# GregVS/Racing-SLAM

Measured on AMD Instinct MI355X. Metric: match+triangulate+local-BA passes/sec @ 2k kpts/frame, 20-KF×10k-pt window, higher is better.
Workload: dtype u8 Hamming (match), f64 (DLT SVD, BA), f32 (gates)

## Files before the change

racing-slam_amd/csrc/common.h:

```cpp
#pragma once
#include <hip/hip_runtime.h>
#include <stdint.h>
#include <stdio.h>
#include <string.h>

#include <string>
#include <vector>

#include "../../include/rsgpu.h"
#include "dev_array.h"

#define RS_WAVE 64

struct rs_prof_slot {
    char name[32];
    int launches;
    std::vector<hipEvent_t> ev;
};

struct rs_arena {
    char* base = nullptr;
    size_t cap = 0, used = 0;
    std::vector<void*> retired;
};
// ... 4 lines not shown
    hipStream_t stream = nullptr;
    std::string err;
    void* ws = nullptr;
    size_t ws_bytes = 0;
    int32_t* grp_zero_ptr = nullptr;
    int grp_zero_n = 0;
    size_t ws_dirty_hi = 0;
    void* pinned = nullptr;
    size_t pinned_bytes = 0;
    rs_arena stage_dev, stage_pin;
    std::vector<rs_pending_download> stage_down;
    bool prof_on = false;
    std::vector<rs_prof_slot> prof;
    void* comm = nullptr;
    int n_ranks = 1;
    int rank = 0;
    struct rs_local_group* local = nullptr;
    void* ba_cache = nullptr;
    const void* ba_trace = nullptr;
    int ba_trace_n = 0;
    int ba_stats[8] = {0, 0, 0, 0, 0, 0, 0, 0};
    int ba_item = 0;
    int ba_batch_item = 0;
    int ba_band_mode = 0;
    int ba_s_replicas = 0;
    int ba_handoff_timeout_us = 4000;
    const double* ba_cams = nullptr;
    int ba_cams_n = 0;
    int ba_sets = 0;
    int n_cu = 256;
    int ba_fuse_mode = 0;
    int k2_mode = 0;
    int k2_grid = 1;
    int ba_imu_mode = 0;
    int ba_batch_mode = 0;
    int bow_score_mode = 0;
    int loop_verify_streams = 0;
    int gftt_round_launches = 12;
    std::vector<rs_context*> batch_lanes;
    std::vector<hipStream_t> batch_streams;
    rs_dev_array<unsigned long long> prop;
    hipEvent_t sync_ev = nullptr;
    void* tri_pin = nullptr;
    int tri_ticket = 0;
    rs_dev_array<uint2> k1_top;
};

struct rs_frame {
    rs_context* ctx = nullptr;
    int n = 0;
    rs_dev_block block;
    rs_pin_block pin;
    float* d_kp = nullptr; uint8_t* d_desc = nullptr; int32_t* d_kd = nullptr;
    uint8_t* d_matched = nullptr;
    void* d_packed = nullptr;
    int kd_root = -1;
    int cap = 0;
    uint32_t* d_rank = nullptr;
    int32_t* d_n = nullptr;
    int32_t* h_n = nullptr;
    int32_t* d_kp_point = nullptr;
    rs_dev_array<unsigned char> grid;
    int grid_w = 0, grid_h = 0;
    bool grid_built = false;
    bool finite = false;
};
// ... 131 lines not shown
```

racing-slam_amd/csrc/context.hip:

```cpp
#include <dlfcn.h>
#include <stdarg.h>
#include <stdlib.h>

#include "common.h"

int rs_fail(rs_context* ctx, int code, const char* fmt, ...)
{
    char buf[512];
    va_list ap;
    va_start(ap, fmt);
    vsnprintf(buf, sizeof buf, fmt, ap);
    va_end(ap);
    if (ctx) ctx->err = buf;
    else fprintf(stderr, "rsgpu: %s\n", buf);
    return code;
}

extern "C" int rs_abi_version(void) { return RSGPU_ABI_VERSION; }

extern "C" int rs_context_create(int device_id, rs_context** out)
{
    if (!out) return RS_ERR_INVALID;
    *out = nullptr;
    int n = 0;
// ... 109 lines not shown
    if (strcmp(name, "ba_item_landmarks") == 0) {
        if (value != 0 && (value < 32 || value > 64 || value % 8)) return rs_fail(ctx, RS_ERR_INVALID, "ba_item_landmarks must be 0 (default) or 32, 40, 48, 56, 64");
        ctx->ba_item = value;
        return RS_OK;
    }
    if (strcmp(name, "ba_batch_item_landmarks") == 0) {
        if (value != 0 && (value < 32 || value > 64 || value % 8)) return rs_fail(ctx, RS_ERR_INVALID, "ba_batch_item_landmarks must be 0 (default) or 32, 40, 48, 56, 64");
        ctx->ba_batch_item = value;
        return RS_OK;
    }
    if (strcmp(name, "ba_band_mode") == 0) {
        if (value < 0 || value > 2) return rs_fail(ctx, RS_ERR_INVALID, "ba_band_mode must be 0 (banded factorisation where the reduced matrix is block-banded), 1 (always the general blocked one) or 2 (banded, one workgroup instead of two sides)");
        ctx->ba_band_mode = value;
        return RS_OK;
    }
    if (strcmp(name, "ba_s_replicas") == 0) {
        if (value != 0 && value != 1 && value != 2 && value != 4 && value != 8) return rs_fail(ctx, RS_ERR_INVALID, "ba_s_replicas must be 0 (default), 1, 2, 4 or 8");
        ctx->ba_s_replicas = value;
        return RS_OK;
    }
    if (strcmp(name, "ba_handoff_timeout_us") == 0) {
        if (value < 1 || value > 1000000) return rs_fail(ctx, RS_ERR_INVALID, "ba_handoff_timeout_us must be 1 .. 1000000");
        ctx->ba_handoff_timeout_us = value;
        return RS_OK;
    }
    if (strcmp(name, "k2_mode") == 0) {
        if (value < 0 || value > 1) return rs_fail(ctx, RS_ERR_INVALID, "k2_mode must be 0 (eight lanes per map point where possible) or 1 (one lane per point)");
        ctx->k2_mode = value;
        return RS_OK;
    }
    if (strcmp(name, "k2_grid") == 0) {
        if (value < 0 || value > 1) return rs_fail(ctx, RS_ERR_INVALID, "k2_grid must be 1 (the cell-grid kernel where the frame has a usable grid) or 0 (never)");
        ctx->k2_grid = value;
        return RS_OK;
    }
    if (strcmp(name, "ba_batch_mode") == 0) {
        if (value < 0 || value > 1) return rs_fail(ctx, RS_ERR_INVALID, "ba_batch_mode must be 0 (grid where possible) or 1 (lanes)");
        ctx->ba_batch_mode = value;
        return RS_OK;
    }
    if (strcmp(name, "bow_score_mode") == 0) {
        if (value < 0 || value > 1) return rs_fail(ctx, RS_ERR_INVALID, "bow_score_mode must be 0 (dense word table) or 1 (binary search)");
        ctx->bow_score_mode = value;
        return RS_OK;
    }
    if (strcmp(name, "loop_verify_streams") == 0) {
        if (value < 0 || value > 1) return rs_fail(ctx, RS_ERR_INVALID, "loop_verify_streams must be 0 (one child context per candidate) or 1 (the context stream)");
        ctx->loop_verify_streams = value;
        return RS_OK;
    }
    if (strcmp(name, "gftt_round_launches") == 0) {
        if (value < 0 || value > GFTT_ROUNDS_KNOB) return rs_fail(ctx, RS_ERR_INVALID, "gftt_round_launches must be 0 .. 12 (default 12)");
        ctx->gftt_round_launches = value;
        return RS_OK;
    }
    return rs_fail(ctx, RS_ERR_INVALID, "unknown option %s", name);
}

extern "C" int rs_context_synchronize(rs_context* ctx)
{
    if (!ctx) return RS_ERR_INVALID;
    RS_HIP(ctx, hipStreamSynchronize(ctx->stream));
    return RS_OK;
}

extern "C" const char* rs_last_error(const rs_context* ctx) { return ctx ? ctx->err.c_str() : "null context"; }
// ... 489 lines not shown
```

racing-slam_amd/csrc/tracks.hip:

```cpp
#include "point_core.h"

struct TrackParams {
    TriParams tri;
    float min_parallax_cosine;
    float rotation_factor;
    int kf_pose;
};

#define K6_TABLE_POSES 512
#define K6_BATCH 4

__global__ __launch_bounds__(64) void k6_tracks(const float2* __restrict__ track_uv, const uint8_t* __restrict__ skip,
                                               const int32_t* __restrict__ sight_ptr,
                                               const int32_t* __restrict__ sight_pose,
                                               const float2* __restrict__ sight_uv, const float* __restrict__ poses,
                                               int n_tracks, int n_table, TrackParams prm, uint8_t* __restrict__ status,
                                               float* __restrict__ xyz, float* __restrict__ parallax_cos,
                                               float* __restrict__ required_cos, const float* __restrict__ required_by_pose)
{
    extern __shared__ float kp_rows[];
    for (int i = threadIdx.x; i < n_table; i += blockDim.x) {
        float T[16], KP[12];
        load_pose(poses, i, T);
        projection_rows(prm.tri, T, KP);
#pragma unroll
        for (int k = 0; k < 12; k++) kp_rows[12 * i + k] = KP[k];
    }
    __syncthreads();
    const int t = blockIdx.x * blockDim.x + threadIdx.x;
    if (t >= n_tracks) return;
    const int s0 = sight_ptr[t], s1 = sight_ptr[t + 1];
    uint8_t st = 0;
    float X[3] = {0.f, 0.f, 0.f}, pc = 0.f, rc = 0.f;
    if (s1 > s0 && !(skip && skip[t])) {
        float Tf[16], Tk[16];
        load_pose(poses, sight_pose[s0], Tf);
        load_pose(poses, prm.kf_pose, Tk);
        const bool ok = dlt_one(sight_uv[s0], track_uv[t], Tf, Tk, prm.tri, X);
        if (ok) {
            bool consistent = true;
            if (n_table > 0) {
                for (int s = s0; s < s1 && consistent; s += K6_BATCH) {
                    int ip[K6_BATCH];
                    float2 px[K6_BATCH];
#pragma unroll
                    for (int u = 0; u < K6_BATCH; u++) { const int su = min(s + u, s1 - 1); ip[u] = sight_pose[su]; px[u] = sight_uv[su]; }
#pragma unroll
                    for (int u = 0; u < K6_BATCH; u++) {
                        float KP[12];
                        const int iu = min(max(ip[u], 0), n_table - 1);
#pragma unroll
                        for (int k = 0; k < 12; k++) KP[k] = kp_rows[12 * iu + k];
                        const float2 pr = project_rows_f32(KP, X);
                        const float dx = pr.x - px[u].x, dy = pr.y - px[u].y;
                        if (sqrtf(dx * dx + dy * dy) > prm.tri.max_reprojection_error) consistent = false;
                    }
                }
            } else
            for (int s = s0; s < s1; s++) {
                float Ts[16];
                load_pose(poses, sight_pose[s], Ts);
                const float2 pr = project_f32(prm.tri, Ts, X);
                const float2 px = sight_uv[s];
                const float dx = pr.x - px.x, dy = pr.y - px.y;
                if (sqrtf(dx * dx + dy * dy) > prm.tri.max_reprojection_error) { consistent = false; break; }
            }
            if (!consistent) {
                st = 2;
            } else {
                float cf[3], ck[3];
                camera_center_f32(Tf, cf);
                camera_center_f32(Tk, ck);
                float a[3] = {cf[0] - X[0], cf[1] - X[1], cf[2] - X[2]};
                float b[3] = {ck[0] - X[0], ck[1] - X[1], ck[2] - X[2]};
                normalize3f(a);
                normalize3f(b);
                float tr[3];
#pragma unroll
                for (int i = 0; i < 3; i++) {
                    const float rk[3] = {Tk[4 * i], Tk[4 * i + 1], Tk[4 * i + 2]};
                    const float rf[3] = {Tf[4 * i], Tf[4 * i + 1], Tf[4 * i + 2]};
                    tr[i] = dot3f(rk, rf);
                }
                const float trace = (tr[0] + tr[1]) + tr[2];
                float cosine = (trace - 1.0f) / 2.0f;
                cosine = cosine < -1.0f ? -1.0f : cosine;
                cosine = cosine > 1.0f ? 1.0f : cosine;
                st = 1;
                pc = dot3f(a, b);
                if (required_by_pose) {
                    rc = required_by_pose[sight_pose[s0]];
                } else {
                    const float turned = acosf(cosine);
                    const float need = cosf(prm.rotation_factor * turned);
                    rc = prm.min_parallax_cosine < need ? prm.min_parallax_cosine : need;
                }
            }
        }
    }
    status[t] = st;
    xyz[3 * (size_t)t + 0] = X[0]; xyz[3 * (size_t)t + 1] = X[1]; xyz[3 * (size_t)t + 2] = X[2];
    parallax_cos[t] = pc;
    required_cos[t] = rc;
}

#define K6B_CH 8
#define K6B_REJ_LDS 2048
#define K6B_FIELD 21

__device__ __forceinline__ bool k6_before(float kj, float ki, int j, int i)
{
    return (kj < ki) || (!(ki < kj) && !(kj < ki) && ((kj == kj) == (ki == ki)) && j < i) || ((kj == kj) && !(ki == ki));
}

__device__ __forceinline__ unsigned long long k6_block_exclusive_scan64(unsigned long long v, unsigned long long* total)
{
    __shared__ unsigned long long k6_scan_w[16];
    const int lane = threadIdx.x & 63, wave = threadIdx.x >> 6, nw = (blockDim.x + 63) >> 6;
    unsigned long long x = v;
#pragma unroll
    for (int off = 1; off < 64; off <<= 1) {
        const unsigned long long t = __shfl_up(x, off, 64);
        if (lane >= off) x += t;
    }
    if (lane == 63) k6_scan_w[wave] = x;
    __syncthreads();
    unsigned long long pre = 0, tot = 0;
    for (int w = 0; w < nw; w++) { const unsigned long long c = k6_scan_w[w]; if (w < wave) pre += c; tot += c; }
    __syncthreads();
    *total = tot;
    return pre + x - v;
}

template <int CH>
__device__ __forceinline__ void k6_select_held(const uint8_t* __restrict__ status, const float* __restrict__ pcs,
                                               const float* __restrict__ rcs, int lo, int hi, int min_new_points,
                                               int32_t* __restrict__ accepted, int32_t* __restrict__ inconsistent,
// ... 98 lines not shown
                                     const int32_t* d_sight_ptr, const int32_t* d_sight_pose,
                                     const float* d_sight_uv, const float* d_poses, int n_poses, int kf_pose,
                                     const float h_intrinsics[4], float any_parallax_cosine,
                                     float max_reprojection_error, float min_parallax_cosine,
                                     float rotation_parallax_factor, int min_new_points, uint8_t* d_status,
                                     float* d_xyz, float* d_parallax_cos, float* d_required_cos,
                                     int32_t* d_accepted, int32_t* d_inconsistent, int32_t* d_counts,
                                     const float* d_required_by_pose)
{
    if (!ctx) return RS_ERR_INVALID;
    if (n_tracks < 0 || n_poses < 0) return rs_fail(ctx, RS_ERR_INVALID, "negative size");
    if (!d_counts) return rs_fail(ctx, RS_ERR_INVALID, "null counts");
    RS_HIP(ctx, hipSetDevice(ctx->device));
    if (n_tracks == 0) {
        RS_HIP(ctx, hipMemsetAsync(d_counts, 0, 3 * sizeof(int32_t), ctx->stream));
        return RS_OK;
    }
    if (!d_track_uv || !d_sight_ptr || !d_sight_pose || !d_sight_uv || !d_poses || !h_intrinsics || !d_status ||
        !d_xyz || !d_parallax_cos || !d_required_cos || !d_accepted || !d_inconsistent)
        return rs_fail(ctx, RS_ERR_INVALID, "null pointer");
    if (kf_pose < 0 || kf_pose >= n_poses) return rs_fail(ctx, RS_ERR_INVALID, "key-frame pose index out of range");
    if ((uintptr_t)d_poses & 15) return rs_fail(ctx, RS_ERR_INVALID, "poses must be 16-byte aligned");
    void* ws = nullptr;
    int rc = rs_workspace(ctx, sizeof(int32_t) * (size_t)n_tracks, &ws);
    if (rc) return rc;
    TrackParams prm;
    prm.tri = {h_intrinsics[0], h_intrinsics[1], h_intrinsics[2], h_intrinsics[3], any_parallax_cosine, max_reprojection_error};
    prm.min_parallax_cosine = min_parallax_cosine;
    prm.rotation_factor = rotation_parallax_factor;
    prm.kf_pose = kf_pose;
    {
        rs_prof_scope ps(ctx, "K6_tracks");
        const int n_table = n_poses <= K6_TABLE_POSES ? n_poses : 0;
        hipLaunchKernelGGL(k6_tracks, dim3((n_tracks + 63) / 64), dim3(64), sizeof(float) * 12 * (size_t)n_table, ctx->stream,
                           (const float2*)d_track_uv, d_skip, d_sight_ptr, d_sight_pose, (const float2*)d_sight_uv, d_poses, n_tracks, n_table, prm,
                           d_status, d_xyz, d_parallax_cos, d_required_cos, d_required_by_pose);
    }
    {
        rs_prof_scope ps(ctx, "K6b_select");
        hipLaunchKernelGGL(k6_select, dim3(1), dim3(1024), 0, ctx->stream, d_status, d_parallax_cos, d_required_cos,
                           n_tracks, min_new_points, d_accepted, d_inconsistent, (int32_t*)ws, d_counts);
    }
    RS_HIP(ctx, hipGetLastError());
    return RS_OK;
}

__global__ __launch_bounds__(256) void k12_point_errors(const float* __restrict__ pos, const int32_t* __restrict__ obs_ptr,
                                                        const int32_t* __restrict__ obs_pose,
                                                        const float2* __restrict__ obs_uv, const float* __restrict__ poses,
                                                        int n_points, TriParams k, float max_mean_error,
                                                        float* __restrict__ mean_err, uint8_t* __restrict__ cull,
                                                        double* __restrict__ sums)
{
    const int p = blockIdx.x * blockDim.x + threadIdx.x;
    double esum = 0.0, ecnt = 0.0;
    if (p < n_points) {
        const float X[3] = {pos[3 * (size_t)p], pos[3 * (size_t)p + 1], pos[3 * (size_t)p + 2]};
        const int o0 = obs_ptr[p], o1 = obs_ptr[p + 1];
        const float err = point_error_sum_f32(k, poses, obs_pose, obs_uv, nullptr, X, o0, o1, &esum);
        const int cnt = o1 - o0;
        ecnt = (double)cnt;
        float mean;
        const bool c = point_cull_rule_f32(err, cnt, max_mean_error, &mean);
        mean_err[p] = mean;
        cull[p] = c ? 1 : 0;
    }
    esum = wave_sum_f64(esum);
// ... 186 lines not shown
```

racing-slam_amd/csrc/tri_core.h:

```cpp
#pragma once
#include "common.h"

struct TriParams {
    float fx, fy, cx, cy;
    float min_parallax_cosine, max_reprojection_error;
};

__device__ __forceinline__ double cv_hypot(double a, double b)
{
    a = fabs(a);
    b = fabs(b);
    if (a > b) { b /= a; return a * sqrt(1 + b * b); }
    if (b > 0) { a /= b; return b * sqrt(1 + a * a); }
    return 0;
}

__device__ __forceinline__ float dot3f(const float* a, const float* b) { return (a[0] * b[0] + a[1] * b[1]) + a[2] * b[2]; }

__device__ __forceinline__ void normalize3f(float* v)
{
    const float n = dot3f(v, v);
    if (n > 0.0f) {
        const float s = sqrtf(n);
        v[0] = v[0] / s; v[1] = v[1] / s; v[2] = v[2] / s;
    }
}

__device__ __forceinline__ float det3f(float a, float b, float c, float d, float e, float f, float g, float h, float i)
{
    return (a * (e * i - f * h) - b * (d * i - f * g)) + c * (d * h - e * g);
}

__device__ __forceinline__ void inverse_translation(const float* T, float* c)
{
    const float M0 = det3f(T[1], T[2], T[3], T[5], T[6], T[7], T[9], T[10], T[11]);
    const float M1 = det3f(T[0], T[2], T[3], T[4], T[6], T[7], T[8], T[10], T[11]);
    const float M2 = det3f(T[0], T[1], T[3], T[4], T[5], T[7], T[8], T[9], T[11]);
    const float M3 = det3f(T[0], T[1], T[2], T[4], T[5], T[6], T[8], T[9], T[10]);
    const float det = (-T[12] * M0 + T[13] * M1) + (-T[14] * M2 + T[15] * M3);
    c[0] = -M0 / det;
    c[1] = M1 / det;
    c[2] = -M2 / det;
}

__device__ __forceinline__ void projection_rows(const TriParams& k, const float* T, float* P)
{
#pragma unroll
    for (int j = 0; j < 4; j++) {
        P[0 * 4 + j] = (k.fx * T[0 * 4 + j] + 0.0f * T[1 * 4 + j]) + k.cx * T[2 * 4 + j];
        P[1 * 4 + j] = (0.0f * T[0 * 4 + j] + k.fy * T[1 * 4 + j]) + k.cy * T[2 * 4 + j];
        P[2 * 4 + j] = (0.0f * T[0 * 4 + j] + 0.0f * T[1 * 4 + j]) + 1.0f * T[2 * 4 + j];
    }
}

#define JACOBI_PAIR(i, j)                                                                      \
    {                                                                                          \
        double a = W[i], p = 0, b = W[j];                                                      \
        _Pragma("unroll") for (int k = 0; k < 4; k++) p += At[i][k] * At[j][k];                \
        if (!(fabs(p) <= eps * sqrt(a * b))) {                                                 \
            p *= 2;                                                                            \
            const double beta = a - b, gamma = cv_hypot(p, beta);                              \
            double c, s;                                                                       \
            if (beta < 0) {                                                                    \
                const double delta = (gamma - beta) * 0.5;                                     \
                s = sqrt(delta / gamma);                                                       \
                c = p / (gamma * s * 2);                                                       \
            } else {                                                                           \
                c = sqrt((gamma + beta) / (gamma * 2));                                        \
                s = p / (gamma * c * 2);                                                       \
            }                                                                                  \
            a = 0; b = 0;                                                                      \
            _Pragma("unroll") for (int k = 0; k < 4; k++) {                                    \
                const double t0 = c * At[i][k] + s * At[j][k];                                 \
                const double t1 = -s * At[i][k] + c * At[j][k];                                \
                At[i][k] = t0; At[j][k] = t1;                                                  \
                a += t0 * t0; b += t1 * t1;                                                    \
            }                                                                                  \
            W[i] = a; W[j] = b;                                                                \
            changed = true;                                                                    \
            _Pragma("unroll") for (int k = 0; k < 4; k++) {                                    \
                const double t0 = c * Vt[i][k] + s * Vt[j][k];                                 \
                const double t1 = -s * Vt[i][k] + c * Vt[j][k];                                \
                Vt[i][k] = t0; Vt[j][k] = t1;                                                  \
            }                                                                                  \
        }                                                                                      \
    }

__device__ __forceinline__ void load_pose(const float* __restrict__ poses, int idx, float* T)
{
    const float4* a = (const float4*)(poses + 16 * (size_t)idx);
#pragma unroll
    for (int r = 0; r < 4; r++) {
        const float4 v = a[r];
        T[4 * r] = v.x; T[4 * r + 1] = v.y; T[4 * r + 2] = v.z; T[4 * r + 3] = v.w;
    }
}

__device__ __forceinline__ float2 project_rows_f32(const float* KP, const float* X)
{
    float uvw[3];
#pragma unroll
    for (int i = 0; i < 3; i++)
        uvw[i] = (KP[4 * i] * X[0] + KP[4 * i + 1] * X[1]) + (KP[4 * i + 2] * X[2] + KP[4 * i + 3] * 1.0f);
    if (uvw[2] < 0.0f) return make_float2(-1.0f, -1.0f);
    return make_float2(uvw[0] / uvw[2], uvw[1] / uvw[2]);
}

__device__ __forceinline__ float2 project_f32(const TriParams& k, const float* T, const float* X)
{
    float KP[12];
    projection_rows(k, T, KP);
    return project_rows_f32(KP, X);
}

__device__ __forceinline__ void camera_center_f32(const float* T, float* c)
{
    const float t[3] = {T[3], T[7], T[11]};
#pragma unroll
    for (int i = 0; i < 3; i++) {
        const float a[3] = {-T[0 * 4 + i], -T[1 * 4 + i], -T[2 * 4 + i]};
        c[i] = dot3f(a, t);
    }
}

__device__ __forceinline__ double wave_sum_f64(double v)
{
#pragma unroll
    for (int off = 32; off > 0; off >>= 1) v += __shfl_xor(v, off, 64);
    return v;
}

__device__ __forceinline__ bool dlt_one(const float2 p1, const float2 p2, const float* T1, const float* T2,
                                        const TriParams& prm, float* Xout)
{
    double At[4][4], Vt[4][4], W[4];
    {
        float P1[12], P2[12];
        projection_rows(prm, T1, P1);
        projection_rows(prm, T2, P2);
#pragma unroll
        for (int k = 0; k < 4; k++) {
            At[k][0] = (double)p1.x * (double)P1[8 + k] - (double)P1[k];
            At[k][1] = (double)p1.y * (double)P1[8 + k] - (double)P1[4 + k];
            At[k][2] = (double)p2.x * (double)P2[8 + k] - (double)P2[k];
            At[k][3] = (double)p2.y * (double)P2[8 + k] - (double)P2[4 + k];
        }
    }
    const double eps = 2.220446049250313e-16 * 10;
#pragma unroll
    for (int r = 0; r < 4; r++) {
        double sd = 0;
#pragma unroll
        for (int k = 0; k < 4; k++) sd += At[r][k] * At[r][k];
        W[r] = sd;
#pragma unroll
        for (int k = 0; k < 4; k++) Vt[r][k] = (r == k) ? 1.0 : 0.0;
    }
    for (int iter = 0; iter < 30; iter++) {
        bool changed = false;
        JACOBI_PAIR(0, 1) JACOBI_PAIR(0, 2) JACOBI_PAIR(0, 3)
        JACOBI_PAIR(1, 2) JACOBI_PAIR(1, 3) JACOBI_PAIR(2, 3)
        if (!changed) break;
    }
#pragma unroll
    for (int r = 0; r < 4; r++) {
        double sd = 0;
#pragma unroll
        for (int k = 0; k < 4; k++) sd += At[r][k] * At[r][k];
        W[r] = sqrt(sd);
    }
#pragma unroll
    for (int a = 0; a < 3; a++) {
        int j = a;
#pragma unroll
        for (int k = a + 1; k < 4; k++)
            if (W[j] < W[k]) j = k;
#pragma unroll
        for (int k = a + 1; k < 4; k++) {
            if (j == k) {
                const double tw = W[a]; W[a] = W[k]; W[k] = tw;
#pragma unroll
                for (int m = 0; m < 4; m++) { const double tv = Vt[a][m]; Vt[a][m] = Vt[k][m]; Vt[k][m] = tv; }
            }
        }
    }
    const float h0 = (float)Vt[3][0], h1 = (float)Vt[3][1], h2 = (float)Vt[3][2], h3 = (float)Vt[3][3];
    float X[3] = {h0 / h3, h1 / h3, h2 / h3};
    Xout[0] = X[0]; Xout[1] = X[1]; Xout[2] = X[2];

    bool ok = true;
    float c1[3], c2[3];
#pragma unroll
    for (int r = 0; r < 3; r++) {
        c1[r] = (T1[4 * r] * X[0] + T1[4 * r + 1] * X[1]) + (T1[4 * r + 2] * X[2] + T1[4 * r + 3] * 1.0f);
        c2[r] = (T2[4 * r] * X[0] + T2[4 * r + 1] * X[1]) + (T2[4 * r + 2] * X[2] + T2[4 * r + 3] * 1.0f);
    }
    if (c1[2] < 0.0f || c2[2] < 0.0f) ok = false;
    float o1[3], o2[3];
    inverse_translation(T1, o1);
    inverse_translation(T2, o2);
    float a[3] = {o1[0] - X[0], o1[1] - X[1], o1[2] - X[2]};
    float b[3] = {o2[0] - X[0], o2[1] - X[1], o2[2] - X[2]};
    normalize3f(a);
    normalize3f(b);
    if (dot3f(a, b) > prm.min_parallax_cosine) ok = false;
    const float w1 = (0.0f * c1[0] + 0.0f * c1[1]) + 1.0f * c1[2];
    const float w2 = (0.0f * c2[0] + 0.0f * c2[1]) + 1.0f * c2[2];
    const float i1x = ((prm.fx * c1[0] + 0.0f * c1[1]) + prm.cx * c1[2]) / w1;
    const float i1y = ((0.0f * c1[0] + prm.fy * c1[1]) + prm.cy * c1[2]) / w1;
    const float i2x = ((prm.fx * c2[0] + 0.0f * c2[1]) + prm.cx * c2[2]) / w2;
    const float i2y = ((0.0f * c2[0] + prm.fy * c2[1]) + prm.cy * c2[2]) / w2;
    const float e1x = i1x - p1.x, e1y = i1y - p1.y, e2x = i2x - p2.x, e2y = i2y - p2.y;
    const float err1 = sqrtf(e1x * e1x + e1y * e1y);
    const float err2 = sqrtf(e2x * e2x + e2y * e2y);
    if (err1 > prm.max_reprojection_error || err2 > prm.max_reprojection_error) ok = false;
    return ok;
}
```

racing-slam_amd/csrc/triangulate.hip:

```cpp
#include "tri_core.h"

__device__ __forceinline__ void k4_triangulate_body(
    const float2* __restrict__ uv1, const float2* __restrict__ uv2, int n,
    const float* __restrict__ poses, const int32_t* __restrict__ idx1, const int32_t* __restrict__ idx2,
    const int32_t* __restrict__ gather1, const int32_t* __restrict__ gather2, const int32_t* __restrict__ d_n,
    TriParams prm, float* __restrict__ xyz, uint8_t* __restrict__ keep)
{
    const int i = blockIdx.x * blockDim.x + threadIdx.x;
    if (d_n) n = min(n, *d_n);
    if (i >= n) return;
    float T1[16], T2[16];
    {
        const float4* a = (const float4*)(poses + 16 * (size_t)(idx1 ? idx1[i] : 0));
        const float4* b = (const float4*)(poses + 16 * (size_t)(idx2 ? idx2[i] : 1));
#pragma unroll
        for (int r = 0; r < 4; r++) {
            const float4 va = a[r], vb = b[r];
            T1[4 * r] = va.x; T1[4 * r + 1] = va.y; T1[4 * r + 2] = va.z; T1[4 * r + 3] = va.w;
            T2[4 * r] = vb.x; T2[4 * r + 1] = vb.y; T2[4 * r + 2] = vb.z; T2[4 * r + 3] = vb.w;
        }
    }
    const float2 p1 = uv1[gather1 ? gather1[i] : i], p2 = uv2[gather2 ? gather2[i] : i];
    float X[3];
    const bool ok = dlt_one(p1, p2, T1, T2, prm, X);
    xyz[3 * (size_t)i + 0] = X[0];
    xyz[3 * (size_t)i + 1] = X[1];
    xyz[3 * (size_t)i + 2] = X[2];
    keep[i] = ok ? 1 : 0;
}

template <int CH>
__device__ __forceinline__ void k4_compact_held(const uint8_t* __restrict__ keep, const float* __restrict__ xyz, int lo, int hi,
                                                const int32_t* __restrict__ d_n, int32_t* __restrict__ out_index,
                                                float* __restrict__ out_xyz, int32_t* __restrict__ out_count)
{
    uint8_t k[CH];
    float x[CH][3];
#pragma unroll
    for (int u = 0; u < CH; u++) {
        const int i = max(min(lo + u, hi - 1), 0);
        k[u] = keep[i];
        x[u][0] = xyz[3 * (size_t)i + 0]; x[u][1] = xyz[3 * (size_t)i + 1]; x[u][2] = xyz[3 * (size_t)i + 2];
    }
    const int live = d_n ? min(hi, *d_n) : hi;
    int cnt = 0;
#pragma unroll
    for (int u = 0; u < CH; u++) cnt += (lo + u < live && k[u] != 0) ? 1 : 0;
    int total;
    int off = rs_block_exclusive_scan(cnt, &total);
#pragma unroll
    for (int u = 0; u < CH; u++) {
        if (lo + u >= live || k[u] == 0) continue;
        out_index[off] = lo + u;
        out_xyz[3 * (size_t)off + 0] = x[u][0];
        out_xyz[3 * (size_t)off + 1] = x[u][1];
        out_xyz[3 * (size_t)off + 2] = x[u][2];
        off++;
    }
    if (threadIdx.x == 0) *out_count = total;
}

// ... 22 lines not shown
#pragma unroll
        for (int u = 0; u < 16; u++) cnt += (i0 + u < hi && k[u] != 0) ? 1 : 0;
    }
    int total;
    int off = rs_block_exclusive_scan(cnt, &total);
    for (int i0 = lo; i0 < hi; i0 += 8) {
        uint8_t k[8];
        float x[8][3];
#pragma unroll
        for (int u = 0; u < 8; u++) {
            const int i = min(i0 + u, hi - 1);
            k[u] = keep[i];
            x[u][0] = xyz[3 * (size_t)i + 0]; x[u][1] = xyz[3 * (size_t)i + 1]; x[u][2] = xyz[3 * (size_t)i + 2];
        }
#pragma unroll
        for (int u = 0; u < 8; u++) {
            if (i0 + u >= hi || k[u] == 0) continue;
            out_index[off] = i0 + u;
            out_xyz[3 * (size_t)off + 0] = x[u][0];
            out_xyz[3 * (size_t)off + 1] = x[u][1];
            out_xyz[3 * (size_t)off + 2] = x[u][2];
            off++;
        }
    }
    if (threadIdx.x == 0) *out_count = total;
}

__global__ __launch_bounds__(64) void k4_triangulate(
    const float2* __restrict__ uv1, const float2* __restrict__ uv2, int n,
    const float* __restrict__ poses, const int32_t* __restrict__ idx1, const int32_t* __restrict__ idx2,
    const int32_t* __restrict__ gather1, const int32_t* __restrict__ gather2, const int32_t* __restrict__ d_n,
    TriParams prm, float* __restrict__ xyz, uint8_t* __restrict__ keep)
{
    k4_triangulate_body(uv1, uv2, n, poses, idx1, idx2, gather1, gather2, d_n, prm, xyz, keep);
}

__global__ __launch_bounds__(1024) void k4_compact(const uint8_t* __restrict__ keep, const float* __restrict__ xyz, int n,
                                                   const int32_t* __restrict__ d_n, int32_t* __restrict__ out_index,
                                                   float* __restrict__ out_xyz, int32_t* __restrict__ out_count)
{
    k4_compact_body(keep, xyz, n, d_n, out_index, out_xyz, out_count);
}

__global__ __launch_bounds__(64) void k4_triangulate_pairs(
    const float2* __restrict__ kp1, int n1, const float2* __restrict__ kp2, int n2, int stride,
    const float* __restrict__ poses, const int32_t* __restrict__ match_train, const int32_t* __restrict__ match_query,
    const int32_t* __restrict__ d_n, TriParams prm, float* __restrict__ xyz, uint8_t* __restrict__ keep)
{
    const size_t b = blockIdx.y;
    k4_triangulate_body(kp1 + b * n1, kp2 + b * n2, stride, poses + b * 32, nullptr, nullptr, match_train + b * stride,
                        match_query + b * stride, d_n + b, prm, xyz + b * stride * 3, keep + b * stride);
}

__global__ __launch_bounds__(1024) void k4_compact_pairs(const uint8_t* __restrict__ keep, const float* __restrict__ xyz,
                                                         int stride, const int32_t* __restrict__ d_n,
                                                         int32_t* __restrict__ out_index, float* __restrict__ out_xyz,
                                                         int32_t* __restrict__ out_count)
{
    const size_t b = blockIdx.x;
    k4_compact_body(keep + b * stride, xyz + b * stride * 3, stride, d_n + b, out_index + b * stride,
                    out_xyz + b * stride * 3, out_count + b);
}

static int tri_launch(rs_context* ctx, const float* d_uv1, const float* d_uv2, int n, const float* d_poses,
                      int n_poses, const int32_t* d_pose_idx1, const int32_t* d_pose_idx2,
                      const int32_t* g1, const int32_t* g2, const int32_t* d_n, const float h_intrinsics[4],
                      float min_parallax_cosine, float max_reprojection_error, float* d_xyz, uint8_t* d_keep,
                      int32_t* d_out_index, float* d_out_xyz, int32_t* d_out_count)
{
    if (!ctx) return RS_ERR_INVALID;
    if (n < 0) return rs_fail(ctx, RS_ERR_INVALID, "negative n");
    if (!d_out_count) return rs_fail(ctx, RS_ERR_INVALID, "null out_count");
    RS_HIP(ctx, hipSetDevice(ctx->device));
    if (n == 0) {
        RS_HIP(ctx, hipMemsetAsync(d_out_count, 0, sizeof(int32_t), ctx->stream));
        return RS_OK;
    }
    if (!d_uv1 || !d_uv2 || !d_poses || !h_intrinsics || !d_xyz || !d_keep || !d_out_index || !d_out_xyz)
        return rs_fail(ctx, RS_ERR_INVALID, "null pointer");
    if ((!d_pose_idx1 || !d_pose_idx2) && n_poses < 2) return rs_fail(ctx, RS_ERR_INVALID, "need two poses");
    if ((uintptr_t)d_poses & 15) return rs_fail(ctx, RS_ERR_INVALID, "poses must be 16-byte aligned");
    TriParams prm = {h_intrinsics[0], h_intrinsics[1], h_intrinsics[2], h_intrinsics[3], min_parallax_cosine,
                     max_reprojection_error};
    {
        rs_prof_scope ps(ctx, "K4_triangulate_dlt");
        hipLaunchKernelGGL(k4_triangulate, dim3((n + 63) / 64), dim3(64), 0, ctx->stream, (const float2*)d_uv1,
                           (const float2*)d_uv2, n, d_poses, d_pose_idx1, d_pose_idx2, g1, g2, d_n, prm, d_xyz, d_keep);
    }
    {
        rs_prof_scope ps(ctx, "K4b_compact");
        hipLaunchKernelGGL(k4_compact, dim3(1), dim3(1024), 0, ctx->stream, d_keep, d_xyz, n, d_n, d_out_index,
                           d_out_xyz, d_out_count);
    }
    RS_HIP(ctx, hipGetLastError());
    return RS_OK;
}

extern "C" int rs_triangulate(rs_context* ctx, const float* d_uv1, const float* d_uv2, int n,
                              const float* d_poses, int n_poses, const int32_t* d_pose_idx1,
                              const int32_t* d_pose_idx2, const float h_intrinsics[4],
                              float min_parallax_cosine, float max_reprojection_error, float* d_xyz,
                              uint8_t* d_keep, int32_t* d_out_index, float* d_out_xyz, int32_t* d_out_count)
{
    return tri_launch(ctx, d_uv1, d_uv2, n, d_poses, n_poses, d_pose_idx1, d_pose_idx2, nullptr, nullptr, nullptr,
                      h_intrinsics, min_parallax_cosine, max_reprojection_error, d_xyz, d_keep, d_out_index,
                      d_out_xyz, d_out_count);
}

#define RS_TRI_SMALL 256
struct TriPoses { float T1[16], T2[16]; };
struct TriSmallOut { volatile int flag; int count; int pad[2]; int32_t index[RS_TRI_SMALL]; float xyz[RS_TRI_SMALL * 3]; };

__global__ __launch_bounds__(RS_TRI_SMALL) void k4_small(const float2* __restrict__ uv , int n,
                                                         float2 a0, float2 b0, TriPoses ps, TriParams prm, TriSmallOut* __restrict__ out, int ticket)
{
    const int i = threadIdx.x;
    bool ok = false;
    float X[3] = {0.f, 0.f, 0.f};
    if (i < n) {
        const float2 p1 = n == 1 ? a0 : uv[i], p2 = n == 1 ? b0 : uv[n + i];
// ... 139 lines not shown
```

Measured before the change: 2118.

## Split DLT Jacobi SVD across four lanes per item when the GPU is underfilled

```diff
diff --git a/racing-slam_amd/csrc/common.h b/racing-slam_amd/csrc/common.h
--- a/racing-slam_amd/csrc/common.h
+++ b/racing-slam_amd/csrc/common.h
@@ -60,6 +60,7 @@
     int ba_fuse_mode = 0;
     int k2_mode = 0;
     int k2_grid = 1;
+    int dlt_form = 0;
     int ba_imu_mode = 0;
     int ba_batch_mode = 0;
     int bow_score_mode = 0;
diff --git a/racing-slam_amd/csrc/context.hip b/racing-slam_amd/csrc/context.hip
--- a/racing-slam_amd/csrc/context.hip
+++ b/racing-slam_amd/csrc/context.hip
@@ -165,6 +165,11 @@
     if (strcmp(name, "k2_grid") == 0) {
         if (value < 0 || value > 1) return rs_fail(ctx, RS_ERR_INVALID, "k2_grid must be 1 (the cell-grid kernel where the frame has a usable grid) or 0 (never)");
         ctx->k2_grid = value;
+        return RS_OK;
+    }
+    if (strcmp(name, "dlt_form") == 0) {
+        if (value < 0 || value > 2) return rs_fail(ctx, RS_ERR_INVALID, "dlt_form must be 0 (four lanes per item while the chip has idle SIMDs for them), 1 (always one lane per item) or 2 (always four)");
+        ctx->dlt_form = value;
         return RS_OK;
     }
     if (strcmp(name, "ba_batch_mode") == 0) {
diff --git a/racing-slam_amd/csrc/jacobi_coeff.h b/racing-slam_amd/csrc/jacobi_coeff.h
--- /dev/null
+++ b/racing-slam_amd/csrc/jacobi_coeff.h
@@ -0,0 +1,57 @@
+#pragma once
+#include <math.h>
+
+#ifndef RS_HD
+#if defined(__HIPCC__) || defined(__CUDACC__)
+#define RS_HD __host__ __device__ __forceinline__
+#else
+#define RS_HD inline
+#endif
+#endif
+
+RS_HD double cv_hypot(double a, double b)
+{
+    a = fabs(a);
+    b = fabs(b);
+    const bool swap = a > b;
+    const double hi = swap ? a : b, lo = swap ? b : a;
+    const double q = lo / hi;
+    const double r = hi * sqrt(1 + q * q);
+    return (swap || b > 0) ? r : 0;
+}
+
+RS_HD void jacobi_coeff(double p, double a, double b, double* c, double* s)
+{
+    p *= 2;
+    const double beta = a - b, gamma = cv_hypot(p, beta);
+    const bool neg = beta < 0;
+    const double num = neg ? (gamma - beta) * 0.5 : (gamma + beta);
+    const double den = neg ? gamma : gamma * 2;
+    const double r = sqrt(num / den);
+    const double o = p / (gamma * r * 2);
+    *s = neg ? r : o;
+    *c = neg ? o : r;
+}
+
+RS_HD double cv_hypot_branched(double a, double b)
+{
+    a = fabs(a);
+    b = fabs(b);
+    if (a > b) { b /= a; return a * sqrt(1 + b * b); }
+    if (b > 0) { a /= b; return b * sqrt(1 + a * a); }
+    return 0;
+}
+
+RS_HD void jacobi_coeff_branched(double p, double a, double b, double* c, double* s)
+{
+    p *= 2;
+    const double beta = a - b, gamma = cv_hypot_branched(p, beta);
+    if (beta < 0) {
+        const double delta = (gamma - beta) * 0.5;
+        *s = sqrt(delta / gamma);
+        *c = p / (gamma * *s * 2);
+    } else {
+        *c = sqrt((gamma + beta) / (gamma * 2));
+        *s = p / (gamma * *c * 2);
+    }
+}
diff --git a/racing-slam_amd/csrc/tracks.hip b/racing-slam_amd/csrc/tracks.hip
--- a/racing-slam_amd/csrc/tracks.hip
+++ b/racing-slam_amd/csrc/tracks.hip
@@ -10,11 +10,12 @@
 #define K6_TABLE_POSES 512
 #define K6_BATCH 4
 
-__global__ __launch_bounds__(64) void k6_tracks(const float2* __restrict__ track_uv, const uint8_t* __restrict__ skip,
+template <int LANES>
+__device__ __forceinline__ void k6_tracks_body(const float2* __restrict__ track_uv, const uint8_t* __restrict__ skip,
                                                const int32_t* __restrict__ sight_ptr,
                                                const int32_t* __restrict__ sight_pose,
                                                const float2* __restrict__ sight_uv, const float* __restrict__ poses,
-                                               int n_tracks, int n_table, TrackParams prm, uint8_t* __restrict__ status,
+                                               int n_tracks, int n_table, const TrackParams& prm, uint8_t* __restrict__ status,
                                                float* __restrict__ xyz, float* __restrict__ parallax_cos,
                                                float* __restrict__ required_cos, const float* __restrict__ required_by_pose)
 {
@@ -27,7 +28,7 @@
         for (int k = 0; k < 12; k++) kp_rows[12 * i + k] = KP[k];
     }
     __syncthreads();
-    const int t = blockIdx.x * blockDim.x + threadIdx.x;
+    const int t = (blockIdx.x * blockDim.x + threadIdx.x) / LANES, q = threadIdx.x % LANES;
     if (t >= n_tracks) return;
     const int s0 = sight_ptr[t], s1 = sight_ptr[t + 1];
     uint8_t st = 0;
@@ -36,17 +37,18 @@
         float Tf[16], Tk[16];
         load_pose(poses, sight_pose[s0], Tf);
         load_pose(poses, prm.kf_pose, Tk);
-        const bool ok = dlt_one(sight_uv[s0], track_uv[t], Tf, Tk, prm.tri, X);
+        const bool ok = LANES == 4 ? dlt_quad(q, sight_uv[s0], track_uv[t], Tf, Tk, prm.tri, X)
+                                   : dlt_one(sight_uv[s0], track_uv[t], Tf, Tk, prm.tri, X);
         if (ok) {
             bool consistent = true;
             if (n_table > 0) {
                 for (int s = s0; s < s1 && consistent; s += K6_BATCH) {
-                    int ip[K6_BATCH];
-                    float2 px[K6_BATCH];
-#pragma unroll
-                    for (int u = 0; u < K6_BATCH; u++) { const int su = min(s + u, s1 - 1); ip[u] = sight_pose[su]; px[u] = sight_uv[su]; }
-#pragma unroll
-                    for (int u = 0; u < K6_BATCH; u++) {
+                    int ip[K6_BATCH / LANES];
+                    float2 px[K6_BATCH / LANES];
+#pragma unroll
+                    for (int u = 0; u < K6_BATCH / LANES; u++) { const int su = min(s + LANES * u + q, s1 - 1); ip[u] = sight_pose[su]; px[u] = sight_uv[su]; }
+#pragma unroll
+                    for (int u = 0; u < K6_BATCH / LANES; u++) {
                         float KP[12];
                         const int iu = min(max(ip[u], 0), n_table - 1);
 #pragma unroll
@@ -55,15 +57,18 @@
                         const float dx = pr.x - px[u].x, dy = pr.y - px[u].y;
                         if (sqrtf(dx * dx + dy * dy) > prm.tri.max_reprojection_error) consistent = false;
                     }
+                    if (LANES == 4) consistent = !quad_any(!consistent);
                 }
             } else
-            for (int s = s0; s < s1; s++) {
+            for (int s = s0; s < s1 && consistent; s += LANES) {
                 float Ts[16];
-                load_pose(poses, sight_pose[s], Ts);
+                const int su = min(s + q, s1 - 1);
+                load_pose(poses, sight_pose[su], Ts);
                 const float2 pr = project_f32(prm.tri, Ts, X);
-                const float2 px = sight_uv[s];
+                const float2 px = sight_uv[su];
                 const float dx = pr.x - px.x, dy = pr.y - px.y;
-                if (sqrtf(dx * dx + dy * dy) > prm.tri.max_reprojection_error) { consistent = false; break; }
+                if (sqrtf(dx * dx + dy * dy) > prm.tri.max_reprojection_error) consistent = false;
+                if (LANES == 4) consistent = !quad_any(!consistent);
             }
             if (!consistent) {
                 st = 2;
@@ -98,11 +103,22 @@
             }
         }
     }
+    if (q != 0) return;
     status[t] = st;
     xyz[3 * (size_t)t + 0] = X[0]; xyz[3 * (size_t)t + 1] = X[1]; xyz[3 * (size_t)t + 2] = X[2];
     parallax_cos[t] = pc;
     required_cos[t] = rc;
 }
+
+#define K6_ARGS const float2* __restrict__ track_uv, const uint8_t* __restrict__ skip, const int32_t* __restrict__ sight_ptr,             \
+                const int32_t* __restrict__ sight_pose, const float2* __restrict__ sight_uv, const float* __restrict__ poses, int n_tracks, \
+                int n_table, TrackParams prm, uint8_t* __restrict__ status, float* __restrict__ xyz, float* __restrict__ parallax_cos,      \
+                float* __restrict__ required_cos, const float* __restrict__ required_by_pose
+#define K6_PASS track_uv, skip, sight_ptr, sight_pose, sight_uv, poses, n_tracks, n_table, prm, status, xyz, parallax_cos, required_cos, required_by_pose
+__global__ __launch_bounds__(64) void k6_tracks(K6_ARGS) { k6_tracks_body<1>(K6_PASS); }
+__global__ __launch_bounds__(256) void k6_tracks_quad(K6_ARGS) { k6_tracks_body<4>(K6_PASS); }
+#undef K6_ARGS
+#undef K6_PASS
 
 #define K6B_CH 8
 #define K6B_REJ_LDS 2048
@@ -267,7 +283,8 @@
     {
         rs_prof_scope ps(ctx, "K6_tracks");
         const int n_table = n_poses <= K6_TABLE_POSES ? n_poses : 0;
-        hipLaunchKernelGGL(k6_tracks, dim3((n_tracks + 63) / 64), dim3(64), sizeof(float) * 12 * (size_t)n_table, ctx->stream,
+        const bool quad = rs_dlt_quad(ctx, n_tracks);
+        hipLaunchKernelGGL(quad ? k6_tracks_quad : k6_tracks, dim3((n_tracks + 63) / 64), dim3(quad ? 256 : 64), sizeof(float) * 12 * (size_t)n_table, ctx->stream,
                            (const float2*)d_track_uv, d_skip, d_sight_ptr, d_sight_pose, (const float2*)d_sight_uv, d_poses, n_tracks, n_table, prm,
                            d_status, d_xyz, d_parallax_cos, d_required_cos, d_required_by_pose);
     }
diff --git a/racing-slam_amd/csrc/tri_core.h b/racing-slam_amd/csrc/tri_core.h
--- a/racing-slam_amd/csrc/tri_core.h
+++ b/racing-slam_amd/csrc/tri_core.h
@@ -1,19 +1,11 @@
 #pragma once
 #include "common.h"
+#include "jacobi_coeff.h"
 
 struct TriParams {
     float fx, fy, cx, cy;
     float min_parallax_cosine, max_reprojection_error;
 };
-
-__device__ __forceinline__ double cv_hypot(double a, double b)
-{
-    a = fabs(a);
-    b = fabs(b);
-    if (a > b) { b /= a; return a * sqrt(1 + b * b); }
-    if (b > 0) { a /= b; return b * sqrt(1 + a * a); }
-    return 0;
-}
 
 __device__ __forceinline__ float dot3f(const float* a, const float* b) { return (a[0] * b[0] + a[1] * b[1]) + a[2] * b[2]; }
 
@@ -58,17 +50,9 @@
         double a = W[i], p = 0, b = W[j];                                                      \
         _Pragma("unroll") for (int k = 0; k < 4; k++) p += At[i][k] * At[j][k];                \
         if (!(fabs(p) <= eps * sqrt(a * b))) {                                                 \
-            p *= 2;                                                                            \
-            const double beta = a - b, gamma = cv_hypot(p, beta);                              \
             double c, s;                                                                       \
-            if (beta < 0) {                                                                    \
-                const double delta = (gamma - beta) * 0.5;                                     \
-                s = sqrt(delta / gamma);                                                       \
-                c = p / (gamma * s * 2);                                                       \
-            } else {                                                                           \
-                c = sqrt((gamma + beta) / (gamma * 2));                                        \
-                s = p / (gamma * c * 2);                                                       \
-            }                                                                                  \
+            if (BRANCHY) jacobi_coeff_branched(p, a, b, &c, &s);                               \
+            else jacobi_coeff(p, a, b, &c, &s);                                                \
             a = 0; b = 0;                                                                      \
             _Pragma("unroll") for (int k = 0; k < 4; k++) {                                    \
                 const double t0 = c * At[i][k] + s * At[j][k];                                 \
@@ -130,61 +114,9 @@
     return v;
 }
 
-__device__ __forceinline__ bool dlt_one(const float2 p1, const float2 p2, const float* T1, const float* T2,
-                                        const TriParams& prm, float* Xout)
-{
-    double At[4][4], Vt[4][4], W[4];
-    {
-        float P1[12], P2[12];
-        projection_rows(prm, T1, P1);
-        projection_rows(prm, T2, P2);
-#pragma unroll
-        for (int k = 0; k < 4; k++) {
-            At[k][0] = (double)p1.x * (double)P1[8 + k] - (double)P1[k];
-            At[k][1] = (double)p1.y * (double)P1[8 + k] - (double)P1[4 + k];
-            At[k][2] = (double)p2.x * (double)P2[8 + k] - (double)P2[k];
-            At[k][3] = (double)p2.y * (double)P2[8 + k] - (double)P2[4 + k];
-        }
-    }
-    const double eps = 2.220446049250313e-16 * 10;
-#pragma unroll
-    for (int r = 0; r < 4; r++) {
-        double sd = 0;
-#pragma unroll
-        for (int k = 0; k < 4; k++) sd += At[r][k] * At[r][k];
-        W[r] = sd;
-#pragma unroll
-        for (int k = 0; k < 4; k++) Vt[r][k] = (r == k) ? 1.0 : 0.0;
-    }
-    for (int iter = 0; iter < 30; iter++) {
-        bool changed = false;
-        JACOBI_PAIR(0, 1) JACOBI_PAIR(0, 2) JACOBI_PAIR(0, 3)
-        JACOBI_PAIR(1, 2) JACOBI_PAIR(1, 3) JACOBI_PAIR(2, 3)
-        if (!changed) break;
-    }
-#pragma unroll
-    for (int r = 0; r < 4; r++) {
-        double sd = 0;
-#pragma unroll
-        for (int k = 0; k < 4; k++) sd += At[r][k] * At[r][k];
-        W[r] = sqrt(sd);
-    }
-#pragma unroll
-    for (int a = 0; a < 3; a++) {
-        int j = a;
-#pragma unroll
-        for (int k = a + 1; k < 4; k++)
-            if (W[j] < W[k]) j = k;
-#pragma unroll
-        for (int k = a + 1; k < 4; k++) {
-            if (j == k) {
-                const double tw = W[a]; W[a] = W[k]; W[k] = tw;
-#pragma unroll
-                for (int m = 0; m < 4; m++) { const double tv = Vt[a][m]; Vt[a][m] = Vt[k][m]; Vt[k][m] = tv; }
-            }
-        }
-    }
-    const float h0 = (float)Vt[3][0], h1 = (float)Vt[3][1], h2 = (float)Vt[3][2], h3 = (float)Vt[3][3];
+__device__ __forceinline__ bool dlt_gates(const float h0, const float h1, const float h2, const float h3, const float2 p1,
+                                          const float2 p2, const float* T1, const float* T2, const TriParams& prm, float* Xout)
+{
     float X[3] = {h0 / h3, h1 / h3, h2 / h3};
     Xout[0] = X[0]; Xout[1] = X[1]; Xout[2] = X[2];
 
@@ -216,3 +148,154 @@
     if (err1 > prm.max_reprojection_error || err2 > prm.max_reprojection_error) ok = false;
     return ok;
 }
+
+template <bool BRANCHY = false>
+__device__ __forceinline__ bool dlt_one(const float2 p1, const float2 p2, const float* T1, const float* T2,
+                                        const TriParams& prm, float* Xout)
+{
+    double At[4][4], Vt[4][4], W[4];
+    {
+        float P1[12], P2[12];
+        projection_rows(prm, T1, P1);
+        projection_rows(prm, T2, P2);
+#pragma unroll
+        for (int k = 0; k < 4; k++) {
+            At[k][0] = (double)p1.x * (double)P1[8 + k] - (double)P1[k];
+            At[k][1] = (double)p1.y * (double)P1[8 + k] - (double)P1[4 + k];
+            At[k][2] = (double)p2.x * (double)P2[8 + k] - (double)P2[k];
+            At[k][3] = (double)p2.y * (double)P2[8 + k] - (double)P2[4 + k];
+        }
+    }
+    const double eps = 2.220446049250313e-16 * 10;
+#pragma unroll
+    for (int r = 0; r < 4; r++) {
+        double sd = 0;
+#pragma unroll
+        for (int k = 0; k < 4; k++) sd += At[r][k] * At[r][k];
+        W[r] = sd;
+#pragma unroll
+        for (int k = 0; k < 4; k++) Vt[r][k] = (r == k) ? 1.0 : 0.0;
+    }
+    for (int iter = 0; iter < 30; iter++) {
+        bool changed = false;
+        JACOBI_PAIR(0, 1) JACOBI_PAIR(0, 2) JACOBI_PAIR(0, 3)
+        JACOBI_PAIR(1, 2) JACOBI_PAIR(1, 3) JACOBI_PAIR(2, 3)
+        if (!changed) break;
+    }
+#pragma unroll
+    for (int r = 0; r < 4; r++) {
+        double sd = 0;
+#pragma unroll
+        for (int k = 0; k < 4; k++) sd += At[r][k] * At[r][k];
+        W[r] = sqrt(sd);
+    }
+#pragma unroll
+    for (int a = 0; a < 3; a++) {
+        int j = a;
+#pragma unroll
+        for (int k = a + 1; k < 4; k++)
+            if (W[j] < W[k]) j = k;
+#pragma unroll
+        for (int k = a + 1; k < 4; k++) {
+            if (j == k) {
+                const double tw = W[a]; W[a] = W[k]; W[k] = tw;
+#pragma unroll
+                for (int m = 0; m < 4; m++) { const double tv = Vt[a][m]; Vt[a][m] = Vt[k][m]; Vt[k][m] = tv; }
+            }
+        }
+    }
+    return dlt_gates((float)Vt[3][0], (float)Vt[3][1], (float)Vt[3][2], (float)Vt[3][3], p1, p2, T1, T2, prm, Xout);
+}
+
+static inline bool rs_dlt_quad(const rs_context* ctx, int n_items)
+{
+    return ctx->dlt_form == 2 || (ctx->dlt_form == 0 && (long long)n_items * 4 <= (long long)ctx->n_cu * 4 * 64);
+}
+
+template <int K> __device__ __forceinline__ int quad_bcast_b32(int v)
+{
+    return __builtin_amdgcn_mov_dpp(v, K | (K << 2) | (K << 4) | (K << 6), 0xf, 0xf, true);
+}
+template <int K> __device__ __forceinline__ double quad_bcast(double v)
+{
+    return __hiloint2double(quad_bcast_b32<K>(__double2hiint(v)), quad_bcast_b32<K>(__double2loint(v)));
+}
+template <int K> __device__ __forceinline__ float quad_bcast(float v) { return __int_as_float(quad_bcast_b32<K>(__float_as_int(v))); }
+
+__device__ __forceinline__ double quad_sum(double x)
+{
+    double s = 0;
+    s += quad_bcast<0>(x); s += quad_bcast<1>(x); s += quad_bcast<2>(x); s += quad_bcast<3>(x);
+    return s;
+}
+
+__device__ __forceinline__ bool quad_any(bool v)
+{
+    int x = v ? 1 : 0;
+    x |= __builtin_amdgcn_mov_dpp(x, 0xB1, 0xf, 0xf, true);
+    x |= __builtin_amdgcn_mov_dpp(x, 0x4E, 0xf, 0xf, true);
+    return x != 0;
+}
+
+#define JACOBI_PAIR_QUAD(i, j)                                                                 \
+    {                                                                                          \
+        const double a = W[i], b = W[j], p = quad_sum(At[i] * At[j]);                          \
+        if (!(fabs(p) <= eps * sqrt(a * b))) {                                                 \
+            double c, s;                                                                       \
+            jacobi_coeff(p, a, b, &c, &s);                                                     \
+            const double t0 = c * At[i] + s * At[j];                                           \
+            const double t1 = -s * At[i] + c * At[j];                                          \
+            At[i] = t0; At[j] = t1;                                                            \
+            W[i] = quad_sum(t0 * t0); W[j] = quad_sum(t1 * t1);                                \
+            changed = true;                                                                    \
+            const double v0 = c * Vt[i] + s * Vt[j];                                           \
+            const double v1 = -s * Vt[i] + c * Vt[j];                                          \
+            Vt[i] = v0; Vt[j] = v1;                                                            \
+        }                                                                                      \
+    }
+
+__device__ __forceinline__ bool dlt_quad(const int q, const float2 p1, const float2 p2, const float* T1, const float* T2,
+                                         const TriParams& prm, float* Xout)
+{
+    double At[4], Vt[4], W[4];
+    {
+        const bool second = (q & 2) != 0, isy = (q & 1) != 0;
+        const float px = second ? (isy ? p2.y : p2.x) : (isy ? p1.y : p1.x);
+        const float k0 = isy ? 0.0f : prm.fx, k1 = isy ? prm.fy : 0.0f, k2 = isy ? prm.cy : prm.cx;
+#pragma unroll
+        for (int k = 0; k < 4; k++) {
+            const float t0 = second ? T2[k] : T1[k], t1 = second ? T2[4 + k] : T1[4 + k], t2 = second ? T2[8 + k] : T1[8 + k];
+            const float Pr = (k0 * t0 + k1 * t1) + k2 * t2;
+            const float P2r = (0.0f * t0 + 0.0f * t1) + 1.0f * t2;
+            At[k] = (double)px * (double)P2r - (double)Pr;
+            Vt[k] = (k == q) ? 1.0 : 0.0;
+        }
+    }
+    const double eps = 2.220446049250313e-16 * 10;
+#pragma unroll
+    for (int r = 0; r < 4; r++) W[r] = quad_sum(At[r] * At[r]);
+    for (int iter = 0; iter < 30; iter++) {
+        bool changed = false;
+        JACOBI_PAIR_QUAD(0, 1) JACOBI_PAIR_QUAD(0, 2) JACOBI_PAIR_QUAD(0, 3)
+        JACOBI_PAIR_QUAD(1, 2) JACOBI_PAIR_QUAD(1, 3) JACOBI_PAIR_QUAD(2, 3)
+        if (!changed) break;
+    }
+#pragma unroll
+    for (int r = 0; r < 4; r++) W[r] = sqrt(quad_sum(At[r] * At[r]));
+#pragma unroll
+    for (int a = 0; a < 3; a++) {
+        int j = a;
+#pragma unroll
+        for (int k = a + 1; k < 4; k++)
+            if (W[j] < W[k]) j = k;
+#pragma unroll
+        for (int k = a + 1; k < 4; k++) {
+            if (j == k) {
+                const double tw = W[a]; W[a] = W[k]; W[k] = tw;
+                const double tv = Vt[a]; Vt[a] = Vt[k]; Vt[k] = tv;
+            }
+        }
+    }
+    const float h = (float)Vt[3];
+    return dlt_gates(quad_bcast<0>(h), quad_bcast<1>(h), quad_bcast<2>(h), quad_bcast<3>(h), p1, p2, T1, T2, prm, Xout);
+}
diff --git a/racing-slam_amd/csrc/triangulate.hip b/racing-slam_amd/csrc/triangulate.hip
--- a/racing-slam_amd/csrc/triangulate.hip
+++ b/racing-slam_amd/csrc/triangulate.hip
@@ -1,5 +1,6 @@
 #include "tri_core.h"
 
+template <bool BRANCHY>
 __device__ __forceinline__ void k4_triangulate_body(
     const float2* __restrict__ uv1, const float2* __restrict__ uv2, int n,
     const float* __restrict__ poses, const int32_t* __restrict__ idx1, const int32_t* __restrict__ idx2,
@@ -22,11 +23,34 @@
     }
     const float2 p1 = uv1[gather1 ? gather1[i] : i], p2 = uv2[gather2 ? gather2[i] : i];
     float X[3];
-    const bool ok = dlt_one(p1, p2, T1, T2, prm, X);
+    const bool ok = dlt_one<BRANCHY>(p1, p2, T1, T2, prm, X);
     xyz[3 * (size_t)i + 0] = X[0];
     xyz[3 * (size_t)i + 1] = X[1];
     xyz[3 * (size_t)i + 2] = X[2];
     keep[i] = ok ? 1 : 0;
+}
+
+__global__ __launch_bounds__(64) void k4_triangulate_quad(
+    const float2* __restrict__ uv1, const float2* __restrict__ uv2, int n,
+    const float* __restrict__ poses, const int32_t* __restrict__ idx1, const int32_t* __restrict__ idx2,
+    const int32_t* __restrict__ gather1, const int32_t* __restrict__ gather2, const int32_t* __restrict__ d_n,
+    TriParams prm, float* __restrict__ xyz, uint8_t* __restrict__ keep)
+{
+    const int i = blockIdx.x * 16 + (threadIdx.x >> 2), q = threadIdx.x & 3;
+    if (d_n) n = min(n, *d_n);
+    if (i >= n) return;
+    float T1[16], T2[16];
+    load_pose(poses, idx1 ? idx1[i] : 0, T1);
+    load_pose(poses, idx2 ? idx2[i] : 1, T2);
+    const float2 p1 = uv1[gather1 ? gather1[i] : i], p2 = uv2[gather2 ? gather2[i] : i];
+    float X[3];
+    const bool ok = dlt_quad(q, p1, p2, T1, T2, prm, X);
+    if (q == 0) {
+        xyz[3 * (size_t)i + 0] = X[0];
+        xyz[3 * (size_t)i + 1] = X[1];
+        xyz[3 * (size_t)i + 2] = X[2];
+        keep[i] = ok ? 1 : 0;
+    }
 }
 
 template <int CH>
@@ -115,7 +139,7 @@
     const int32_t* __restrict__ gather1, const int32_t* __restrict__ gather2, const int32_t* __restrict__ d_n,
     TriParams prm, float* __restrict__ xyz, uint8_t* __restrict__ keep)
 {
-    k4_triangulate_body(uv1, uv2, n, poses, idx1, idx2, gather1, gather2, d_n, prm, xyz, keep);
+    k4_triangulate_body<false>(uv1, uv2, n, poses, idx1, idx2, gather1, gather2, d_n, prm, xyz, keep);
 }
 
 __global__ __launch_bounds__(1024) void k4_compact(const uint8_t* __restrict__ keep, const float* __restrict__ xyz, int n,
@@ -131,7 +155,7 @@
     const int32_t* __restrict__ d_n, TriParams prm, float* __restrict__ xyz, uint8_t* __restrict__ keep)
 {
     const size_t b = blockIdx.y;
-    k4_triangulate_body(kp1 + b * n1, kp2 + b * n2, stride, poses + b * 32, nullptr, nullptr, match_train + b * stride,
+    k4_triangulate_body<true>(kp1 + b * n1, kp2 + b * n2, stride, poses + b * 32, nullptr, nullptr, match_train + b * stride,
                         match_query + b * stride, d_n + b, prm, xyz + b * stride * 3, keep + b * stride);
 }
 
@@ -167,8 +191,9 @@
                      max_reprojection_error};
     {
         rs_prof_scope ps(ctx, "K4_triangulate_dlt");
-        hipLaunchKernelGGL(k4_triangulate, dim3((n + 63) / 64), dim3(64), 0, ctx->stream, (const float2*)d_uv1,
-                           (const float2*)d_uv2, n, d_poses, d_pose_idx1, d_pose_idx2, g1, g2, d_n, prm, d_xyz, d_keep);
+        const bool quad = rs_dlt_quad(ctx, n);
+        hipLaunchKernelGGL(quad ? k4_triangulate_quad : k4_triangulate, dim3(quad ? (n + 15) / 16 : (n + 63) / 64), dim3(64), 0, ctx->stream,
+                           (const float2*)d_uv1, (const float2*)d_uv2, n, d_poses, d_pose_idx1, d_pose_idx2, g1, g2, d_n, prm, d_xyz, d_keep);
     }
     {
         rs_prof_scope ps(ctx, "K4b_compact");
```

Measured after the change: 2149 (median of 6 runs). Within noise of the previous version (+1.4%).
